# xxlong0/NeuralUDF

Measured on AMD Instinct MI355X. Metric: ray-samples/sec (train step), higher is better.
Workload: dtype f32 emulated on the 16-bit matrix pipe, f32 accumulate, f32 state / epilogues / optimizer.  Forward-order sweeps (UDF value, input gradient, colour / NeRF forward): f16x2 (x = hi + 2^-11 lo in fp16, 3 fp16 MFMA products, correction terms in their own accumulator).  Backward sweeps (tangent, adjoint

## Files before the change

### neuraludf_amd/csrc/gemm_tn_f32_mfma.hip

```cpp
#include "nudf_common.h"
#include "../../include/nudf.h"
#include <stdio.h>
#include <stdlib.h>
#include <string.h>
#include <type_traits>

#define BM 128
#define BN 128
#define BK 32
#define LDT (BM + 4)
#define T_TILE (BK * LDT)
#define TN_MAX_TILES 64
#define TN_WS_TILE (BM * BN + BM)
#define TNF_RETIRED (2 | 4)
#define TNF_NO_EPILOGUE 2
#define TNF_NO_BIAS 4
#define TNF_ATOMICS 8
#define TNF_UNIFORM_CHUNKS 16
#define TNF_NO_QUADRANTS 32
#define TNF_NO_XCD_MAP 64
#define TNF_NO_INTERLEAVE 128
#define TNF_NO_PACK16 256
#define TNF_NO_SPLIT_IMAGE 512
#define TNF_GENERIC_STAGE 2048
#define TNF_WIDE 1024

typedef float f32x8 __attribute__((ext_vector_type(8)));
typedef __bf16 bf16x8 __attribute__((ext_vector_type(8)));

struct TnTile {
  int blk_start;
  int rows_per_block;
  short prob, ti, tj;
  short layout;
  short n;
  short gfirst;
  short gn;
  short rot;
  int grid_start;
};
struct TnPlan {
  NudfGemmTNProblem prob[NUDF_TN_MAX_PROBLEMS];
  TnTile tile[TN_MAX_TILES + 1];
  int n_tiles, M, prec, flags;
  int grid_blocks;
  short partner[TN_MAX_TILES];
  int assign;
  int wide;
  short unit_tile[TN_MAX_TILES];
  int n_units, unit_chunks;
  float* ws;
  long long* dbg;
  const float* amax_a;
  const float* amax_b;
};

static_assert(sizeof(TnPlan) <= 4096, "TnPlan is passed by value: kernel arguments are limited to 4 KB");

__device__ __forceinline__ int tn_isub(int layout, int wave, int s) {
  return layout == 0 ? s : layout == 1 ? wave : (wave >> 1) * 2 + (s >> 1);
}
__device__ __forceinline__ int tn_jsub(int layout, int wave, int s) {
  return layout == 0 ? wave : layout == 1 ? s : (wave & 1) * 2 + (s & 1);
}

__host__ __device__ __forceinline__ void tn_decode_block(const TnPlan& g, int block, int& t, int& chunk) {
  int gf = 0;
  while (gf + g.tile[gf].gn < g.n_tiles && g.tile[gf + g.tile[gf].gn].grid_start <= block) gf += g.tile[gf].gn;
  const int T = g.tile[gf].gn;
  const int o = block - g.tile[gf].grid_start;
  t = gf;
  chunk = o;
  if (T > 1) {
    const int C = g.tile[gf + 1].blk_start - g.tile[gf].blk_start;
    const int c_hi = o / (8 * T), rem = o - c_hi * 8 * T;
    chunk = c_hi * 8 + (((rem & 7) - g.tile[gf].rot) & 7);
    t = chunk < C ? gf + (rem >> 3) : -1;
  }
}
__device__ __forceinline__ void tn_decode(const TnPlan& g, int& t, int& chunk) { tn_decode_block(g, (int)blockIdx.x, t, chunk); }

__global__ __launch_bounds__(256, 2) void gemm_tn_group_kernel(TnPlan g) {
  __shared__ __attribute__((aligned(16))) float smem[4 * T_TILE];
  float* As = smem;
  float* Bs = smem + 2 * T_TILE;

  const long long t_begin = g.dbg ? (long long)wall_clock64() : 0;
  const long long c_begin = g.dbg ? (long long)__builtin_amdgcn_s_memtime() : 0;
  int t, chunk;
  tn_decode(g, t, chunk);
  if (t < 0) return;
  const TnTile tl = g.tile[t];
  const NudfGemmTNProblem& q = g.prob[tl.prob];
  const int slot_id = tl.blk_start + chunk;

  const int tid = threadIdx.x;
  const int lane = tid & 63;
  const int wave = tid >> 6;
  const int i0 = tl.ti * BM, j0 = tl.tj * BN;
  const int lda = q.lda1, ldb = q.ldb1;
  const int mbeg = chunk * tl.rows_per_block;
  const int mend = min(mbeg + tl.rows_per_block, g.M);
  const int nk = (mend - mbeg + BK - 1) / BK;
  const int nfull = (mend - mbeg) / BK;

  const bool a16 = (q.flags & NUDF_TN_A16) != 0, b16 = (q.flags & NUDF_TN_B16) != 0;
  struct Op { const char* p; size_t rowb, stepb; unsigned poff[4]; int tk, tc, lds_pass; bool blk; };
  auto mk = [&](const float* base, int ld, int c0, bool h, bool blk) {
    Op o;
    const int esz = h ? 2 : 4;
    o.rowb = (size_t)ld * esz;
    o.stepb = (size_t)BK * o.rowb;
    o.blk = blk;
    if (blk) {
      o.tk = tid & 31;
      o.tc = (tid >> 5) * 4;
      o.lds_pass = 32;
      o.p = reinterpret_cast<const char*>(base) + (size_t)mbeg * o.rowb + (size_t)o.tk * 16;
#pragma unroll
      for (int ps = 0; ps < 4; ++ps) o.poff[ps] = (unsigned)(min(c0 + o.tc + 32 * ps, ld - 4) >> 2) * 512u;
    } else {
      o.tk = h ? tid >> 4 : tid >> 5;
      o.tc = h ? (tid & 15) * 8 : (tid & 31) * 4;
      o.lds_pass = (h ? 16 : 8) * LDT;
      const int col = min(c0 + o.tc, ld - (h ? 8 : 4));
      o.p = reinterpret_cast<const char*>(base) + (size_t)(mbeg + o.tk) * o.rowb + (size_t)col * esz;
#pragma unroll
      for (int ps = 0; ps < 4; ++ps) o.poff[ps] = (unsigned)((size_t)ps * (h ? 16 : 8) * o.rowb);
    }
    return o;
  };
  const Op oa = mk(q.A1, lda, i0, a16, (q.flags & NUDF_TN_A_BLK) != 0), ob = mk(q.B1, ldb, j0, b16, (q.flags & NUDF_TN_B_BLK) != 0);
  f32x4 ra[4], rb[4];
  int ld_rows = 0;
  auto load_op = [&](const Op& o, auto H, f32x4 (&r)[4], int kt, bool full) {
    constexpr bool h = decltype(H)::value;
    constexpr int np = h ? 2 : 4, rs = h ? 16 : 8;
    if (full || o.blk) {
      const char* b = o.p + (size_t)kt * o.stepb;
#pragma unroll
      for (int ps = 0; ps < np; ++ps) r[ps] = *reinterpret_cast<const f32x4*>(b + o.poff[ps]);
    } else {
#pragma unroll
      for (int ps = 0; ps < np; ++ps) {
        const ptrdiff_t row = min((ptrdiff_t)kt * BK + ps * rs, (ptrdiff_t)(g.M - 1 - mbeg - o.tk));
        r[ps] = *reinterpret_cast<const f32x4*>(o.p + row * (ptrdiff_t)o.rowb);
      }
    }
  };
  const bool do_bias = (q.dbias != nullptr) && (tl.tj == 0);
  f32x4 bacc = {0.f, 0.f, 0.f, 0.f}, bacc2 = {0.f, 0.f, 0.f, 0.f};
  f32x4 bacc3 = {0.f, 0.f, 0.f, 0.f}, bacc4 = {0.f, 0.f, 0.f, 0.f};
  auto widen = [](const f32x4& raw, f32x4& lo, f32x4& hi) {
    const uint4 u = __builtin_bit_cast(uint4, raw);
    lo = f32x4{__builtin_bit_cast(float, u.x << 16), __builtin_bit_cast(float, u.x & 0xffff0000u),
               __builtin_bit_cast(float, u.y << 16), __builtin_bit_cast(float, u.y & 0xffff0000u)};
    hi = f32x4{__builtin_bit_cast(float, u.z << 16), __builtin_bit_cast(float, u.z & 0xffff0000u),
               __builtin_bit_cast(float, u.w << 16), __builtin_bit_cast(float, u.w & 0xffff0000u)};
  };
  auto store_op = [&](const Op& o, auto H, const f32x4 (&r)[4], float* tile, bool bias) {
    constexpr bool h = decltype(H)::value;
    float* dst = tile + o.tk * LDT + o.tc;
    const f32x4 z = {0.f, 0.f, 0.f, 0.f};
    if constexpr (!h) {
      if (ld_rows >= BK) {
#pragma unroll
        for (int ps = 0; ps < 4; ++ps) *reinterpret_cast<f32x4*>(dst + ps * o.lds_pass) = r[ps];
        if (bias) {
          if (o.blk) { bacc += r[0]; bacc2 += r[1]; bacc3 += r[2]; bacc4 += r[3]; }
          else bacc += (r[0] + r[1]) + (r[2] + r[3]);
        }
        return;
      }
#pragma unroll
      for (int ps = 0; ps < 4; ++ps) {
        const f32x4 v = ((o.blk ? o.tk : ps * 8 + o.tk) < ld_rows) ? r[ps] : z;
        *reinterpret_cast<f32x4*>(dst + ps * o.lds_pass) = v;
        if (bias) {
// ... 1026 lines not shown
      const float x0 = (FULL || r0 + 2 * pp < mend) ? st[2 * pp] : 0.0f;
      const float x1 = (FULL || r0 + 2 * pp + 1 < mend) ? st[2 * pp + 1] : 0.0f;
      unsigned a, b;
      tn_split2_pair(x0, x1, scale, a, b);
      hq[pp >> 2][pp & 3] = a; lq[pp >> 2][pp & 3] = b;
      ps[pp] = x0 + x1;
    }
    if (bias) bias_acc += ((ps[0] + ps[1]) + (ps[2] + ps[3])) + ((ps[4] + ps[5]) + (ps[6] + ps[7]));
    unsigned* dst = tile + ((2 * sg) * 128 + sc) * 4;
    *reinterpret_cast<u32x4*>(dst) = hq[0];
    *reinterpret_cast<u32x4*>(dst + 512) = hq[1];
    *reinterpret_cast<u32x4*>(dst + T3Q) = lq[0];
    *reinterpret_cast<u32x4*>(dst + T3Q + 512) = lq[1];
  };
  auto mma = [&]() {
    const unsigned* as = As + ((lane >> 5) * 128 + (wave >> 1) * 64 + (lane & 31)) * 4;
    const unsigned* bs = Bs + ((lane >> 5) * 128 + (wave & 1) * 64 + (lane & 31)) * 4;
#pragma unroll
    for (int kk = 0; kk < BK3 / 16; ++kk) {
      u32x4 a[2][2], b[2][2];
#pragma unroll
      for (int s2 = 0; s2 < 2; ++s2)
#pragma unroll
        for (int pl = 0; pl < 2; ++pl) {
          a[s2][pl] = *reinterpret_cast<const u32x4*>(as + pl * T3Q + (2 * kk) * 512 + 128 * s2);
          b[s2][pl] = *reinterpret_cast<const u32x4*>(bs + pl * T3Q + (2 * kk) * 512 + 128 * s2);
        }
#pragma unroll
      for (int tt = 0; tt < 3; ++tt) {
        const int qa = (tt == 0) ? 1 : 0, qb = (tt == 1) ? 1 : 0;
#pragma unroll
        for (int j = 0; j < 2; ++j)
#pragma unroll
          for (int i = 0; i < 2; ++i) {
            if (tt < 2)
              acc1[i * 2 + j] = __builtin_amdgcn_mfma_f32_32x32x16_f16(__builtin_bit_cast(f16x8_t, a[i][qa]),
                                                                       __builtin_bit_cast(f16x8_t, b[j][qb]), acc1[i * 2 + j], 0, 0, 0);
            else
              acc[i * 2 + j] = __builtin_amdgcn_mfma_f32_32x32x16_f16(__builtin_bit_cast(f16x8_t, a[i][qa]),
                                                                      __builtin_bit_cast(f16x8_t, b[j][qb]), acc[i * 2 + j], 0, 0, 0);
          }
      }
    }
  };
  typedef std::integral_constant<bool, false> Ragged;
  typedef std::integral_constant<bool, true> Full;
  float sa[16], sb[16], sa2[16], sb2[16];
  if (nk > 0) {
    load(pa, lda, sa, 0);
    load(pb, ldb, sb, 0);
    if (nk > 1) {
      load(pa, lda, sa2, 1);
      load(pb, ldb, sb2, 1);
    }
    store(Ragged{}, sa, 0, As, sca, do_bias);
    store(Ragged{}, sb, 0, Bs, scb, false);
  }
  __syncthreads();
  auto kstep = [&](int kt, float (&la)[16], float (&lb)[16], float (&ua)[16], float (&ub)[16]) {
    if (kt + 2 < nk) {
      load(pa, lda, la, kt + 2);
      load(pb, ldb, lb, kt + 2);
    }
    __builtin_amdgcn_sched_barrier(0);
    mma();
    __builtin_amdgcn_sched_barrier(0);
    __syncthreads();
    if (kt + 1 < nk) {
      store(Ragged{}, ua, kt + 1, As, sca, do_bias);
      store(Ragged{}, ub, kt + 1, Bs, scb, false);
    }
    __syncthreads();
  };
  int kt0 = 0;
  {
    const bool last_ragged = ((mend - mbeg) % BK3) != 0 || mend > g.M;
    const int n_fast = nk - 2 - (last_ragged ? 1 : 0);
    if (n_fast >= 2 && (size_t)(g.M - mbeg) * (size_t)max(q.lda1, q.ldb1) * 4 < ((size_t)1 << 31)) {
      const int sgu = __builtin_amdgcn_readfirstlane(sg);
      const unsigned ca = (unsigned)min(i0 + sc, q.lda1 - 1), cbb = (unsigned)min(j0 + sc, q.ldb1 - 1);
      const __amdgpu_buffer_rsrc_t rsa = __builtin_amdgcn_make_buffer_rsrc(const_cast<float*>(q.A1 + (size_t)mbeg * lda), 0,
                                                                           (int)((size_t)(g.M - mbeg) * lda * 4), 0x00020000);
      const __amdgpu_buffer_rsrc_t rsb = __builtin_amdgcn_make_buffer_rsrc(const_cast<float*>(q.B1 + (size_t)mbeg * ldb), 0,
                                                                           (int)((size_t)(g.M - mbeg) * ldb * 4), 0x00020000);
      const int lda4 = q.lda1 * 4, ldb4 = q.ldb1 * 4;
      int ba = (2 * BK3 + 16 * sgu) * lda4, bb = (2 * BK3 + 16 * sgu) * ldb4;
      const int sa_step = BK3 * lda4, sb_step = BK3 * ldb4;
      auto load_f = [&](__amdgpu_buffer_rsrc_t rs, int so, int ld4, unsigned col, float (&st)[16]) {
#pragma unroll
        for (int r = 0; r < 16; ++r)
          st[r] = __builtin_bit_cast(float, __builtin_amdgcn_raw_buffer_load_b32(rs, (int)(col * 4), so + r * ld4, 0));
      };
      auto fstep = [&](float (&la)[16], float (&lb)[16], float (&ua)[16], float (&ub)[16]) {
        load_f(rsa, ba, lda4, ca, la);
        load_f(rsb, bb, ldb4, cbb, lb);
        ba += sa_step;
        bb += sb_step;
        __builtin_amdgcn_sched_barrier(0);
        mma();
        __builtin_amdgcn_sched_barrier(0);
        __syncthreads();
        store(Full{}, ua, 0, As, sca, do_bias);
        store(Full{}, ub, 0, Bs, scb, false);
        __syncthreads();
      };
      do {
        fstep(sa, sb, sa2, sb2);
        fstep(sa2, sb2, sa, sb);
        kt0 += 2;
      } while (kt0 + 1 < n_fast);
    }
  }
  for (int kt = kt0; kt < nk; kt += 2) {
    kstep(kt, sa, sb, sa2, sb2);
    if (kt + 1 < nk) kstep(kt + 1, sa2, sb2, sa, sb);
  }

  if (g.flags & TNF_NO_EPILOGUE) return;
  float* slot = g.ws ? g.ws + (size_t)slot_id * TN_WS_TILE : nullptr;
  if (do_bias) {
    float* red = reinterpret_cast<float*>(smem);
    red[sg * BM + sc] = bias_acc;
    __syncthreads();
    if (tid < BM) {
      const float sum = red[tid] + red[BM + tid];
      if (slot) slot[BM * BN + tid] = sum;
      else if (i0 + tid < q.NA) atomicAdd(q.dbias + i0 + tid, sum);
    }
  }
  const float unscale = inva * invb;
#pragma unroll
  for (int s4 = 0; s4 < 4; ++s4) {
#pragma unroll
    for (int r = 0; r < 16; ++r) acc[s4][r] = __builtin_fmaf(acc1[s4][r], 1.0f / 2048.0f, acc[s4][r]) * unscale;
    if (slot) {
      float* w = slot + ((wave * 4 + s4) * 64 + lane) * 16;
#pragma unroll
      for (int qd = 0; qd < 4; ++qd) {
        const f32x4 v = {acc[s4][4 * qd], acc[s4][4 * qd + 1], acc[s4][4 * qd + 2], acc[s4][4 * qd + 3]};
        *reinterpret_cast<f32x4*>(w + 4 * qd) = v;
      }
    } else {
      const int col = j0 + 32 * tn_jsub(2, wave, s4) + (lane & 31);
      if (col >= q.NB) continue;
#pragma unroll
      for (int r = 0; r < 16; ++r) {
        const int row = i0 + 32 * tn_isub(2, wave, s4) + (r & 3) + 8 * (r >> 2) + 4 * (lane >> 5);
        if (row < q.NA) atomicAdd(q.C + (size_t)row * q.ldc + col, acc[s4][r]);
      }
    }
  }
}

#define T3WA (4 * 256 * 4)
#define T3WB (4 * 128 * 4)
#define T3W_BUF (3 * T3WA + 3 * T3WB)
__global__ __launch_bounds__(512, 1) void gemm_tn3w_group_kernel(TnPlan g) {
  __shared__ __attribute__((aligned(16))) unsigned smem_w[2 * T3W_BUF];
  const int t = g.unit_tile[blockIdx.x / g.unit_chunks];
  const int chunk = blockIdx.x % g.unit_chunks;
  const int partner = g.partner[t];
  const TnTile tl = g.tile[t];
  const NudfGemmTNProblem& q = g.prob[tl.prob];
  const bool two = partner >= 0;
  const int slot0 = tl.blk_start + chunk;
  const int slot1 = two ? g.tile[partner].blk_start + chunk : slot0;

  const int tid = threadIdx.x;
  const int lane = tid & 63;
  const int wave = tid >> 6;
  const int i0 = tl.ti * BM, j0 = tl.tj * BN;
  const int mbeg = chunk * tl.rows_per_block;
  const int mend = min(mbeg + tl.rows_per_block, g.M);
  const int nk = (mend - mbeg + BK3 - 1) / BK3;
  const int sca = tid & 255, sga = tid >> 8;
  const int scb = tid & 127, sgb = tid >> 7;
  const bool bias_tile = (q.dbias != nullptr) && (tl.tj == 0) && !(g.flags & TNF_NO_BIAS);
  const bool do_bias = bias_tile && (two || sca < BM);
  float bias_acc = 0.0f;
  const bool mm_live = two || wave < 4;

  f32x16 acc[4];
#pragma unroll
  for (int s2 = 0; s2 < 4; ++s2)
#pragma unroll
    for (int r = 0; r < 16; ++r) acc[s2][r] = 0.0f;

  const float* pa = q.A1 + min(i0 + sca, q.lda1 - 1);
  const float* pb = q.B1 + min(j0 + scb, q.ldb1 - 1);
  const size_t lda = (size_t)q.lda1, ldb = (size_t)q.ldb1;
  auto load_a = [&](float (&st)[16], int kt) {
    const int r0 = mbeg + kt * BK3 + 16 * sga;
#pragma unroll
    for (int r = 0; r < 16; ++r) st[r] = pa[(size_t)min(r0 + r, g.M - 1) * lda];
  };
  auto load_b = [&](float (&st)[8], int kt) {
    const int r0 = mbeg + kt * BK3 + 8 * sgb;
#pragma unroll
    for (int r = 0; r < 8; ++r) st[r] = pb[(size_t)min(r0 + r, g.M - 1) * ldb];
  };
  auto store_a = [&](const float (&st)[16], int kt, unsigned* img) {
    const int r0 = mbeg + kt * BK3 + 16 * sga;
    u32x4 hq[2], mq[2], lq[2];
    float ps[8];
#pragma unroll
    for (int pp = 0; pp < 8; ++pp) {
      const float x0 = (r0 + 2 * pp < mend) ? st[2 * pp] : 0.0f;
      const float x1 = (r0 + 2 * pp + 1 < mend) ? st[2 * pp + 1] : 0.0f;
      unsigned a, b, d;
      tn_split3_pair(x0, x1, a, b, d);
      hq[pp >> 2][pp & 3] = a; mq[pp >> 2][pp & 3] = b; lq[pp >> 2][pp & 3] = d;
      ps[pp] = x0 + x1;
    }
    if (do_bias) bias_acc += ((ps[0] + ps[1]) + (ps[2] + ps[3])) + ((ps[4] + ps[5]) + (ps[6] + ps[7]));
    unsigned* dst = img + ((2 * sga) * 256 + sca) * 4;
    *reinterpret_cast<u32x4*>(dst) = hq[0];
    *reinterpret_cast<u32x4*>(dst + 1024) = hq[1];
    *reinterpret_cast<u32x4*>(dst + T3WA) = mq[0];
    *reinterpret_cast<u32x4*>(dst + T3WA + 1024) = mq[1];
    *reinterpret_cast<u32x4*>(dst + 2 * T3WA) = lq[0];
    *reinterpret_cast<u32x4*>(dst + 2 * T3WA + 1024) = lq[1];
  };
  auto store_b = [&](const float (&st)[8], int kt, unsigned* img) {
    const int r0 = mbeg + kt * BK3 + 8 * sgb;
    u32x4 hq, mq, lq;
#pragma unroll
    for (int pp = 0; pp < 4; ++pp) {
      const float x0 = (r0 + 2 * pp < mend) ? st[2 * pp] : 0.0f;
      const float x1 = (r0 + 2 * pp + 1 < mend) ? st[2 * pp + 1] : 0.0f;
      unsigned a, b, d;
      tn_split3_pair(x0, x1, a, b, d);
      hq[pp] = a; mq[pp] = b; lq[pp] = d;
    }
    unsigned* dst = img + 3 * T3WA + (sgb * 128 + scb) * 4;
    *reinterpret_cast<u32x4*>(dst) = hq;
    *reinterpret_cast<u32x4*>(dst + T3WB) = mq;
    *reinterpret_cast<u32x4*>(dst + 2 * T3WB) = lq;
  };
  auto mma = [&](const unsigned* img) {
    const unsigned* as = img + ((lane >> 5) * 256 + (wave >> 1) * 64 + (lane & 31)) * 4;
    const unsigned* bs = img + 3 * T3WA + ((lane >> 5) * 128 + (wave & 1) * 64 + (lane & 31)) * 4;
    u32x4 fa[2][2][3], fb[2][2][3];
    auto ldf = [&](int kk) {
#pragma unroll
      for (int s2 = 0; s2 < 2; ++s2)
#pragma unroll
        for (int pl = 0; pl < 3; ++pl) {
          fa[kk][s2][pl] = *reinterpret_cast<const u32x4*>(as + pl * T3WA + (2 * kk) * 1024 + 128 * s2);
          fb[kk][s2][pl] = *reinterpret_cast<const u32x4*>(bs + pl * T3WB + (2 * kk) * 512 + 128 * s2);
        }
    };
    ldf(0);
#pragma unroll
    for (int kk = 0; kk < BK3 / 16; ++kk) {
      if (kk + 1 < BK3 / 16) ldf(kk + 1);
      __builtin_amdgcn_sched_barrier(0);
#pragma unroll
      for (int tt = 0; tt < 6; ++tt) {
        const int qa = (tt == 0 || tt == 3 || tt == 5) ? 0 : (tt == 1 ? 2 : 1);
        const int qb = (tt == 0) ? 2 : ((tt == 2 || tt == 3) ? 1 : 0);
#pragma unroll
        for (int j = 0; j < 2; ++j)
#pragma unroll
          for (int i = 0; i < 2; ++i)
            acc[i * 2 + j] = __builtin_amdgcn_mfma_f32_32x32x16_bf16(__builtin_bit_cast(bf16x8, fa[kk][i][qa]),
                                                                     __builtin_bit_cast(bf16x8, fb[kk][j][qb]), acc[i * 2 + j], 0, 0, 0);
      }
      __builtin_amdgcn_sched_barrier(0);
    }
  };
  unsigned* buf0 = smem_w;
  unsigned* buf1 = smem_w + T3W_BUF;
  float sa[16], sb[8], sa2[16], sb2[8];
  if (nk > 0) {
    load_a(sa, 0);
    load_b(sb, 0);
    if (nk > 1) {
      load_a(sa2, 1);
      load_b(sb2, 1);
    }
    store_a(sa, 0, buf0);
    store_b(sb, 0, buf0);
  }
  const bool mma_first = wave < 4;
  long long tk_mma = 0, tk_store = 0, tk_load = 0, tk_bar = 0;
  const bool prof = g.dbg != nullptr;
  const long long tk_begin = prof ? (long long)__builtin_amdgcn_s_memtime() : 0;
#define TNW_STAMP(acc_) if (prof) { const long long n_ = (long long)__builtin_amdgcn_s_memtime(); acc_ += n_ - tk_last; tk_last = n_; }
  if (!mma_first && nk > 2) {
    load_a(sa, 2);
    load_b(sb, 2);
  }
  __syncthreads();
  auto kstep = [&](int kt, float (&la)[16], float (&lb)[8], float (&ua)[16], float (&ub)[8], const unsigned* cur, unsigned* nxt) {
    long long tk_last = prof ? (long long)__builtin_amdgcn_s_memtime() : 0;
    if (mma_first) {
      if (kt + 2 < nk) {
        load_a(la, kt + 2);
        load_b(lb, kt + 2);
      }
      __builtin_amdgcn_sched_barrier(0);
      TNW_STAMP(tk_load)
      if (mm_live) mma(cur);
      __builtin_amdgcn_sched_barrier(0);
      TNW_STAMP(tk_mma)
      if (kt + 1 < nk) {
        store_a(ua, kt + 1, nxt);
        store_b(ub, kt + 1, nxt);
      }
      __builtin_amdgcn_sched_barrier(0);
      TNW_STAMP(tk_store)
    } else {
      if (kt + 1 < nk) {
        store_a(ua, kt + 1, nxt);
        store_b(ub, kt + 1, nxt);
      }
      __builtin_amdgcn_sched_barrier(0);
      TNW_STAMP(tk_store)
      if (kt + 3 < nk) {
        load_a(ua, kt + 3);
        load_b(ub, kt + 3);
      }
      __builtin_amdgcn_sched_barrier(0);
      TNW_STAMP(tk_load)
      if (mm_live) mma(cur);
      __builtin_amdgcn_sched_barrier(0);
      TNW_STAMP(tk_mma)
    }
    __builtin_amdgcn_sched_barrier(0);
    __syncthreads();
    TNW_STAMP(tk_bar)
  };
  for (int kt = 0; kt < nk; kt += 2) {
    kstep(kt, sa, sb, sa2, sb2, buf0, buf1);
    if (kt + 1 < nk) kstep(kt + 1, sa2, sb2, sa, sb, buf1, buf0);
  }

#undef TNW_STAMP
  if (prof && lane == 0 && (wave == 0 || wave == 4)) {
    long long* d = g.dbg + 8 * (size_t)blockIdx.x + (wave ? 4 : 0);
    d[0] = ((long long)__builtin_amdgcn_s_memtime() - tk_begin) | ((long long)nk << 40);
    d[1] = tk_mma; d[2] = tk_store | (tk_load << 32); d[3] = tk_bar;
  }
  if (g.flags & TNF_NO_EPILOGUE) return;
  const int tsel = wave >> 2;
  const int vw = 2 * ((wave >> 1) & 1) + (wave & 1);
  float* slot_t[2] = {g.ws ? g.ws + (size_t)slot0 * TN_WS_TILE : nullptr, g.ws ? g.ws + (size_t)slot1 * TN_WS_TILE : nullptr};
  if (bias_tile) {
    float* red = reinterpret_cast<float*>(smem_w);
    red[sga * 256 + sca] = bias_acc;
    __syncthreads();
    if (tid < 256 && (two || tid < BM)) {
      const float sum = red[tid] + red[256 + tid];
      float* sl = slot_t[tid >> 7];
      if (sl) sl[BM * BN + (tid & 127)] = sum;
      else if (i0 + tid < q.NA) atomicAdd(q.dbias + i0 + tid, sum);
    }
  }
  if (!mm_live) return;
#pragma unroll
  for (int s2 = 0; s2 < 4; ++s2) {
    float* slot = slot_t[tsel];
    if (slot) {
      float* w = slot + ((vw * 4 + s2) * 64 + lane) * 16;
#pragma unroll
      for (int qd = 0; qd < 4; ++qd) {
        const f32x4 v = {acc[s2][4 * qd], acc[s2][4 * qd + 1], acc[s2][4 * qd + 2], acc[s2][4 * qd + 3]};
        *reinterpret_cast<f32x4*>(w + 4 * qd) = v;
      }
    } else {
      const int col = j0 + 32 * tn_jsub(2, vw, s2) + (lane & 31);
      if (col >= q.NB) continue;
#pragma unroll
      for (int r = 0; r < 16; ++r) {
        const int row = i0 + 128 * tsel + 32 * tn_isub(2, vw, s2) + (r & 3) + 8 * (r >> 2) + 4 * (lane >> 5);
        if (row < q.NA) atomicAdd(q.C + (size_t)row * q.ldc + col, acc[s2][r]);
      }
    }
  }
}

static int g_tn_flags = -1;
extern "C" int nudf_set_tn_flags(int f) {
  const int old = g_tn_flags < 0 ? 0 : g_tn_flags;
  g_tn_flags = f & ~TNF_RETIRED;
  return old;
}
static long long* g_tn_dbg = nullptr;
extern "C" int nudf_set_tn_debug(void* buf) {
  g_tn_dbg = (long long*)buf;
  return 0;
}
static int tn_flags() {
  if (g_tn_flags < 0) { const char* e = getenv("NUDF_TN_FLAGS"); g_tn_flags = (e ? atoi(e) : 0) & ~TNF_RETIRED; }
  return g_tn_flags;
}

static double tn_cost(int n) {
  static double c[4] = {-1.0, 0, 0, 0};
  if (c[0] < 0) {
    double d[4] = {2.0, 3.0, 3.5, 4.0};
    const char* e = getenv("NUDF_TN_COSTS");
    if (e) sscanf(e, "%lf,%lf,%lf,%lf", &d[0], &d[1], &d[2], &d[3]);
    for (int i = 3; i >= 0; --i) c[i] = d[i];
  }
  return c[n - 1];
}

static int tn_plan(const NudfGemmTNGroup& g, TnPlan& pl) {
  if (g.n_problems <= 0 || g.M <= 0) return 0;
  if (g.n_problems > NUDF_TN_MAX_PROBLEMS) {
    nudf_set_error("nudf_gemm_tn_grouped: too many problems", hipErrorInvalidValue);
    return -1;
  }
  const int flags = tn_flags();
  double cost[TN_MAX_TILES];
  int nt = 0;
  for (int i = 0; i < g.n_problems; ++i) {
    const NudfGemmTNProblem& q = g.prob[i];
    const int ma = (q.flags & NUDF_TN_A16) ? 8 : 4, mb = (q.flags & NUDF_TN_B16) ? 8 : 4;
    {
      const bool ap4 = (q.flags & NUDF_TN_A_P4) != 0, bp4 = (q.flags & NUDF_TN_B_P4) != 0;
      const bool a16 = (q.flags & NUDF_TN_A16) != 0, b16 = (q.flags & NUDF_TN_B16) != 0;
      if ((ap4 && !a16) || (bp4 && !b16) || ((ap4 || bp4) && (g.prec == 0 || g.prec == 3)) || (ap4 && b16 && !bp4) || (bp4 && a16 && !ap4) ||
          ((ap4 || bp4) && (flags & TNF_NO_PACK16)) || ((ap4 || bp4) && g.rows_per_block % 4)) {
        nudf_set_error("nudf_gemm_tn_grouped: a 4-point packed operand is a bf16 operand of the 16-bit MFMA mode "
                       "(NUDF_TN_x16 set, prec != 0, rows_per_block a multiple of 4); a problem's other operand is packed "
                       "as well or fp32", hipErrorInvalidValue);
        return -1;
      }
    }
    if (((q.flags & NUDF_TN_A_BLK) && (q.flags & NUDF_TN_A16)) || ((q.flags & NUDF_TN_B_BLK) && (q.flags & NUDF_TN_B16))) {
      nudf_set_error("nudf_gemm_tn_grouped: the blocked layout is defined for fp32 operands", hipErrorInvalidValue);
      return -1;
    }
    if ((q.lda1 % ma) || (q.ldb1 % mb) || q.NA <= 0 || q.NB <= 0 || q.lda1 < ma || q.ldb1 < mb ||
        (((uintptr_t)q.A1) & 15) || (((uintptr_t)q.B1) & 15)) {
      nudf_set_error("nudf_gemm_tn_grouped: leading dimensions must be multiples of 4, operands 16-byte aligned",
                     hipErrorInvalidValue);
      return -1;
    }
    pl.prob[i] = q;
    const int ti_n = (q.NA + BM - 1) / BM, tj_n = (q.NB + BN - 1) / BN;
    for (int ti = 0; ti < ti_n; ++ti)
      for (int tj = 0; tj < tj_n; ++tj) {
        if (nt >= TN_MAX_TILES) {
          nudf_set_error("nudf_gemm_tn_grouped: more than 64 output tiles of 128 x 128 in one group",
                         hipErrorInvalidValue);
          return -1;
        }
        int li = (q.NA - ti * BM + 31) / 32, lj = (q.NB - tj * BN + 31) / 32;
        if (li > 4) li = 4;
        if (lj > 4) lj = 4;
        TnTile& tl = pl.tile[nt];
        tl.prob = (short)i; tl.ti = (short)ti; tl.tj = (short)tj; tl.rot = 0;
        tl.layout = (short)(li <= lj ? 0 : 1);
        tl.n = (short)(li <= lj ? li : lj);
        if (li == 4 && lj == 4 && !(flags & TNF_NO_QUADRANTS)) tl.layout = 2;
        if (g.prec != 0 || (q.flags & (NUDF_TN_A16 | NUDF_TN_B16))) {
          tl.layout = 2;
          tl.n = 4;
        }
        cost[nt++] = tn_cost(tl.n);
      }
  }
  if (g.workspace && !(flags & TNF_ATOMICS)) {
    for (int i = 0; i < g.n_problems; ++i)
      for (int j = i + 1; j < g.n_problems; ++j) {
        const NudfGemmTNProblem &a = g.prob[i], &b = g.prob[j];
        const float *a0 = a.C, *a1 = a.C + (size_t)(a.NA - 1) * a.ldc + a.NB;
        const float *b0 = b.C, *b1 = b.C + (size_t)(b.NA - 1) * b.ldc + b.NB;
        const bool c_overlap = a0 < b1 && b0 < a1;
        const bool d_overlap = a.dbias && b.dbias && a.dbias < b.dbias + b.NA && b.dbias < a.dbias + a.NA;
        if (c_overlap || d_overlap) {
          nudf_set_error("nudf_gemm_tn_grouped: with a workspace the problems of a group must write disjoint C / dbias "
                         "ranges (the fixed-order reduction is not atomic)", hipErrorInvalidValue);
          return -1;
        }
      }
  }
  pl.n_tiles = nt;
  pl.M = g.M;
  pl.prec = g.prec;
  pl.flags = flags;
  pl.wide = 0;
  int n_units = nt;
  for (int t = 0; t < nt; ++t) pl.partner[t] = -1;
  {
    bool ok = g.prec == 3 && (flags & TNF_WIDE) && !(flags & TNF_NO_SPLIT_IMAGE);
    for (int i = 0; i < g.n_problems && ok; ++i)
      if (g.prob[i].flags & (NUDF_TN_A16 | NUDF_TN_B16 | NUDF_TN_A_BLK | NUDF_TN_B_BLK | NUDF_TN_A_P4 | NUDF_TN_B_P4)) ok = false;
    if (ok) {
      int pairs = 0;
      for (int t = 0; t < nt; ++t) {
        if (pl.partner[t] != -1 || (pl.tile[t].ti & 1)) continue;
        const NudfGemmTNProblem& q = g.prob[pl.tile[t].prob];
        const int tj_n = (q.NB + BN - 1) / BN;
        const int u = t + tj_n;
        if (u < nt && pl.tile[u].prob == pl.tile[t].prob && pl.tile[u].ti == pl.tile[t].ti + 1 && pl.tile[u].tj == pl.tile[t].tj) {
          pl.partner[t] = (short)u;
          pl.partner[u] = -2;
          ++pairs;
        }
      }
      if (4 * pairs >= nt) {
        pl.wide = 1;
        n_units = nt - pairs;
      } else {
        for (int t = 0; t < nt; ++t) pl.partner[t] = -1;
      }
    }
  }
  const int nkt = (g.M + BK - 1) / BK;
  int chunks_of[TN_MAX_TILES];
  int blocks = 0;
  auto layout = [&]() {
    blocks = 0;
    for (int t = 0; t < nt; ++t) {
      pl.tile[t].blk_start = blocks;
      blocks += (g.M + pl.tile[t].rows_per_block - 1) / pl.tile[t].rows_per_block;
    }
    pl.tile[nt].blk_start = blocks;
    pl.tile[nt].gfirst = (short)nt; pl.tile[nt].gn = 1; pl.tile[nt].rot = 0;
    for (int t = 0; t < nt;) {
      int e = t + 1;
      while (!(flags & TNF_NO_XCD_MAP) && e < nt && pl.tile[e].prob == pl.tile[t].prob &&
             pl.tile[e].rows_per_block == pl.tile[t].rows_per_block) ++e;
      for (int k = t; k < e; ++k) { pl.tile[k].gfirst = (short)t; pl.tile[k].gn = (short)(e - t); }
      t = e;
    }
    int load[8] = {0, 0, 0, 0, 0, 0, 0, 0};
    int G = 0;
    for (int t = 0; t < nt; t += pl.tile[t].gn) {
      const int T = pl.tile[t].gn, C = pl.tile[t + 1].blk_start - pl.tile[t].blk_start;
      int rot = 0, size = C;
      if (T == 1) {
        for (int i = 0; i < C; ++i) ++load[(G + i) & 7];
      } else {
        const int w = C & 7;
        for (int x = 0; x < 8; ++x) load[x] += T * (C >> 3);
        if (w) {
          int best = 1 << 30;
          for (int r = 0; r < 8; ++r) {
            int m = 0, sum = 0;
            for (int cl = 0; cl < w; ++cl) { const int l = load[(G + ((cl + r) & 7)) & 7]; m = l > m ? l : m; sum += l; }
            if (m * 4096 + sum < best) { best = m * 4096 + sum; rot = r; }
          }
          for (int cl = 0; cl < w; ++cl) load[(G + ((cl + rot) & 7)) & 7] += T;
        }
        size = ((C + 7) >> 3) * 8 * T;
      }
      for (int k = t; k < t + T; ++k) { pl.tile[k].grid_start = G; pl.tile[k].rot = (short)rot; }
      G += size;
    }
    pl.tile[nt].grid_start = G;
    pl.grid_blocks = G;
    int m = 0;
    for (int x = 0; x < 8; ++x) m = load[x] > m ? load[x] : m;
    return m;
  };
  if (g.rows_per_block > 0) {
    bool any_blk = false;
    for (int i = 0; i < g.n_problems; ++i) any_blk = any_blk || (g.prob[i].flags & (NUDF_TN_A_BLK | NUDF_TN_B_BLK));
    if (any_blk && (g.rows_per_block % 32)) {
      nudf_set_error("nudf_gemm_tn_grouped: rows_per_block must be a multiple of 32 with blocked operands",
                     hipErrorInvalidValue);
      return -1;
    }
    for (int t = 0; t < nt; ++t) pl.tile[t].rows_per_block = g.rows_per_block;
    layout();
  } else {
    static int target0 = -1;
    if (target0 < 0) { const char* e = getenv("NUDF_TNG_BLOCKS"); target0 = e ? atoi(e) : 512; }
    const int max_chunks = nkt / 8 > 0 ? nkt / 8 : 1;
    if (pl.wide) {
      static int target_w = -1;
      if (target_w < 0) { const char* e = getenv("NUDF_TNW_BLOCKS"); target_w = e ? atoi(e) : 256; }
      int n = target_w / n_units;
      if (n < 1) n = 1;
      if (n > max_chunks) n = max_chunks;
      for (int t = 0; t < nt; ++t) chunks_of[t] = n;
      for (int t = 0; t < nt; ++t) pl.tile[t].rows_per_block = ((nkt + chunks_of[t] - 1) / chunks_of[t]) * BK;
      layout();
    } else {
      for (int target = target0;; target -= 8) {
        auto count = [&](double T, bool store) {
          long total = 0;
          for (int t = 0; t < nt; ++t) {
            const double c = ((flags & TNF_UNIFORM_CHUNKS) || g.prec != 0) ? 4.0 : cost[t];
            long n = (long)((c * (double)nkt + T - 1e-9) / T);
            if (n < 1) n = 1;
            if (n > max_chunks) n = max_chunks;
            if (store) chunks_of[t] = (int)n;
            total += n;
          }
          return total;
        };
        double lo = 0.0, hi = 4.0 * nkt;
        if (count(hi, false) <= target) {
          for (int it = 0; it < 60; ++it) {
            const double mid = 0.5 * (lo + hi);
            if (count(mid, false) <= target) hi = mid; else lo = mid;
          }
        }
        count(hi, true);
        for (int t = 0; t < nt; ++t) pl.tile[t].rows_per_block = ((nkt + chunks_of[t] - 1) / chunks_of[t]) * BK;
        const int most = layout();
        if (most <= target0 / 8 || target - 8 < nt || target - 8 < target0 / 2) break;
      }
    }
  }
  pl.n_units = 0;
  pl.unit_chunks = nt > 0 ? pl.tile[1].blk_start - pl.tile[0].blk_start : 1;
  if (pl.wide) {
    for (int t = 0; t < nt; ++t) {
      if (pl.tile[t + 1].blk_start - pl.tile[t].blk_start != pl.unit_chunks) pl.wide = 0;
      if (pl.partner[t] != -2) pl.unit_tile[pl.n_units++] = (short)t;
    }
  }
  return blocks;
}

extern "C" int64_t nudf_gemm_tn_grouped_workspace(const NudfGemmTNGroup* args) {
  TnPlan pl;
  const int blocks = tn_plan(*args, pl);
  pl.dbg = nullptr;
  return blocks <= 0 ? (int64_t)blocks : (int64_t)blocks * TN_WS_TILE;
}

extern "C" int nudf_gemm_tn_grouped_plan(const NudfGemmTNGroup* args, int32_t* out, int capacity) {
  TnPlan pl;
  const int blocks = tn_plan(*args, pl);
  if (blocks <= 0) return blocks;
  for (int b = 0; b < pl.grid_blocks && b < capacity; ++b) {
    int t, chunk;
    tn_decode_block(pl, b, t, chunk);
    if (t < 0) { out[4 * b] = out[4 * b + 1] = out[4 * b + 2] = out[4 * b + 3] = -1; continue; }
    out[4 * b] = pl.tile[t].prob;
    out[4 * b + 1] = pl.tile[t].ti * 256 + pl.tile[t].tj;
    out[4 * b + 2] = chunk;
    out[4 * b + 3] = pl.tile[t].blk_start + chunk;
  }
  return pl.grid_blocks;
}

extern "C" int nudf_gemm_tn_grouped(const NudfGemmTNGroup* args, void* stream) {
  TnPlan pl;
  const int blocks = tn_plan(*args, pl);
  if (blocks == 0) return 0;
  if (blocks < 0) return (int)hipErrorInvalidValue;
  pl.ws = (pl.flags & TNF_ATOMICS) ? nullptr : args->workspace;
  pl.dbg = g_tn_dbg;
  pl.assign = args->assign ? 1 : 0;
  if (pl.assign && !pl.ws) {
    nudf_set_error("nudf_gemm_tn_grouped: assign needs the workspace (two-pass) path", hipErrorInvalidValue);
    return (int)hipErrorInvalidValue;
  }
  if (pl.ws && ((((uintptr_t)pl.ws) & 15) || args->workspace_floats < (int64_t)blocks * TN_WS_TILE)) {
    nudf_set_error("nudf_gemm_tn_grouped: workspace too small or not 16-byte aligned "
                   "(nudf_gemm_tn_grouped_workspace gives the size)", hipErrorInvalidValue);
    return (int)hipErrorInvalidValue;
  }
  bool packed16 = pl.prec != 0 && pl.prec != 3 && !(pl.flags & TNF_NO_PACK16);
  int n16 = 0;
  for (int i = 0; i < args->n_problems && packed16; ++i) {
    const int f = args->prob[i].flags;
    if (f & (NUDF_TN_A_BLK | NUDF_TN_B_BLK)) packed16 = false;
    n16 += ((f & NUDF_TN_A16) ? 1 : 0) + ((f & NUDF_TN_B16) ? 1 : 0);
  }
  if (n16 < args->n_problems) packed16 = false;
  bool any_p4 = false;
  for (int i = 0; i < args->n_problems; ++i) any_p4 = any_p4 || (args->prob[i].flags & (NUDF_TN_A_P4 | NUDF_TN_B_P4));
  if (any_p4) {
    for (int i = 0; i < args->n_problems; ++i)
      if (args->prob[i].flags & (NUDF_TN_A_BLK | NUDF_TN_B_BLK)) {
        nudf_set_error("nudf_gemm_tn_grouped: 4-point packed and blocked operands cannot share a group", hipErrorInvalidValue);
        return (int)hipErrorInvalidValue;
      }
    packed16 = true;
  }
  if (pl.prec == 4) {
    for (int i = 0; i < args->n_problems; ++i)
      if (args->prob[i].flags & (NUDF_TN_A16 | NUDF_TN_B16 | NUDF_TN_A_BLK | NUDF_TN_B_BLK | NUDF_TN_A_P4 | NUDF_TN_B_P4)) {
        nudf_set_error("nudf_gemm_tn_grouped: prec 4 (f16x2) takes fp32 row-major operands", hipErrorInvalidValue);
        return (int)hipErrorInvalidValue;
      }
    pl.amax_a = args->amax_a;
    pl.amax_b = args->amax_b;
    hipLaunchKernelGGL(gemm_tn2_group_kernel, dim3(pl.grid_blocks), dim3(256), 0, (hipStream_t)stream, pl);
    NUDF_CHECK_LAUNCH("nudf_gemm_tn_grouped");
    if (pl.ws) {
      hipLaunchKernelGGL(tn_reduce_kernel, dim3(pl.n_tiles * 17), dim3(256), 0, (hipStream_t)stream, pl);
      NUDF_CHECK_LAUNCH("nudf_gemm_tn_grouped (reduce)");
    }
    return 0;
  }
  bool split3 = pl.prec == 3 && !(pl.flags & TNF_NO_SPLIT_IMAGE);
  for (int i = 0; i < args->n_problems && split3; ++i)
    if (args->prob[i].flags & (NUDF_TN_A16 | NUDF_TN_B16 | NUDF_TN_A_BLK | NUDF_TN_B_BLK | NUDF_TN_A_P4 | NUDF_TN_B_P4)) split3 = false;
  if (split3 && pl.wide)
    hipLaunchKernelGGL(gemm_tn3w_group_kernel, dim3(pl.n_units * pl.unit_chunks), dim3(512), 0, (hipStream_t)stream, pl);
  else if (split3) hipLaunchKernelGGL(gemm_tn3_group_kernel, dim3(pl.grid_blocks), dim3(256), 0, (hipStream_t)stream, pl);
  else if (packed16) hipLaunchKernelGGL(gemm_tn16_group_kernel, dim3(pl.grid_blocks), dim3(256), 0, (hipStream_t)stream, pl);
  else hipLaunchKernelGGL(gemm_tn_group_kernel, dim3(pl.grid_blocks), dim3(256), 0, (hipStream_t)stream, pl);
  NUDF_CHECK_LAUNCH("nudf_gemm_tn_grouped");
  if (pl.ws) {
    hipLaunchKernelGGL(tn_reduce_kernel, dim3(pl.n_tiles * 17), dim3(256), 0, (hipStream_t)stream, pl);
    NUDF_CHECK_LAUNCH("nudf_gemm_tn_grouped (reduce)");
  }
  return 0;
}

extern "C" int nudf_gemm_tn(const NudfGemmTN* args, void* stream) {
  const NudfGemmTN& p = *args;
  if (p.M <= 0 || p.NA <= 0 || p.NB <= 0) return 0;
  NudfGemmTNGroup g;
  memset(&g, 0, sizeof(g));
  g.M = p.M; g.rows_per_block = p.rows_per_block; g.prec = p.prec;
  g.n_problems = p.A2 ? 2 : 1;
  NudfGemmTNProblem& q0 = g.prob[0];
  q0.A1 = p.A1; q0.B1 = p.B1; q0.C = p.C; q0.dbias = p.dbias;
  q0.lda1 = p.lda1; q0.ldb1 = p.ldb1; q0.ldc = p.ldc; q0.NA = p.NA; q0.NB = p.NB;
  if (p.A2) {
    NudfGemmTNProblem& q1 = g.prob[1];
    q1 = q0;
    q1.A1 = p.A2; q1.B1 = p.B2; q1.lda1 = p.lda2; q1.ldb1 = p.ldb2; q1.dbias = nullptr;
  }
  return nudf_gemm_tn_grouped(&g, stream);
}
```

Measured before the change: 19.29 million.

## Add wide f16x2 TN GEMM kernel with buffer loads and transposed LDS reads

Adds a new kernel for the f16x2 (prec 4) weight-gradient TN GEMM. Waves are specialised: half split the A operand into fp16 hi/lo planes and half split B, staging them in a swizzled LDS image. Fragments are read back with ds_read_tr16 transposed loads and fed to 32x32x16 f16 MFMAs, with register double-buffering of global buffer loads. The launcher uses this kernel by default when alignment and size limits allow, keeping the old kernel behind a NARROW flag. The validator now also accepts unaligned leading dimensions for prec 4, which the new kernel rejects and sends back to the old path. The added LDS, register pressure and swizzle logic may lower occupancy.

New measurement: 19.40 million (median of 6 runs). No clear change (+0.6%).

```diff
diff --git a/neuraludf_amd/csrc/gemm_tn_f32_mfma.hip b/neuraludf_amd/csrc/gemm_tn_f32_mfma.hip
--- a/neuraludf_amd/csrc/gemm_tn_f32_mfma.hip
+++ b/neuraludf_amd/csrc/gemm_tn_f32_mfma.hip
@@ -24,6 +24,7 @@
 #define TNF_NO_SPLIT_IMAGE 512
 #define TNF_GENERIC_STAGE 2048
 #define TNF_WIDE 1024
+#define TNF_TN2_NARROW 4096
 
 typedef float f32x8 __attribute__((ext_vector_type(8)));
 typedef __bf16 bf16x8 __attribute__((ext_vector_type(8)));
@@ -1356,6 +1357,197 @@
   }
 }
 
+typedef short s16x4 __attribute__((ext_vector_type(4)));
+typedef short s16x8 __attribute__((ext_vector_type(8)));
+typedef unsigned u32x2_t __attribute__((ext_vector_type(2)));
+typedef __attribute__((address_space(3))) s16x4 lds_s16x4;
+__global__ __launch_bounds__(256, 2) void gemm_tn2w_group_kernel(TnPlan g) {
+  constexpr int BKW = 32;
+  constexpr int PLANE = BKW * 256;
+  __shared__ __attribute__((aligned(16))) unsigned char smem[4 * PLANE];
+  unsigned char* As = smem;
+  unsigned char* Bs = smem + 2 * PLANE;
+
+  int t, chunk;
+  tn_decode(g, t, chunk);
+  if (t < 0) return;
+  const TnTile tl = g.tile[t];
+  const NudfGemmTNProblem& q = g.prob[tl.prob];
+  const int slot_id = tl.blk_start + chunk;
+
+  const int tid = threadIdx.x;
+  const int lane = tid & 63;
+  const int wave = tid >> 6;
+  const int i0 = tl.ti * BM, j0 = tl.tj * BN;
+  const int mbeg = chunk * tl.rows_per_block;
+  const int mend = min(mbeg + tl.rows_per_block, g.M);
+  const int nk = (mend - mbeg + BKW - 1) / BKW;
+  const int c4 = tid & 31, hh = lane >> 5;
+  const int wu = __builtin_amdgcn_readfirstlane(wave);
+  const bool opb = wu >= 2;
+  const int wh = wu & 1;
+  const bool tile_bias = (q.dbias != nullptr) && (tl.tj == 0);
+  const bool do_bias = tile_bias && !opb;
+  f32x4 bias_acc = {0.0f, 0.0f, 0.0f, 0.0f};
+  float sca, inva, scb, invb;
+  tn_scale_of(g.amax_a, sca, inva);
+  tn_scale_of(g.amax_b, scb, invb);
+  const float scale = opb ? scb : sca;
+
+  f32x16 acc[4], acc1[4];
+#pragma unroll
+  for (int s4 = 0; s4 < 4; ++s4)
+#pragma unroll
+    for (int r = 0; r < 16; ++r) { acc[s4][r] = 0.0f; acc1[s4][r] = 0.0f; }
+
+  const int ldo = opb ? q.ldb1 : q.lda1;
+  const int ld4 = ldo * 4;
+  const int col4 = min((opb ? j0 : i0) + 4 * c4, ldo - 4) * 4;
+  const __amdgpu_buffer_rsrc_t rs = __builtin_amdgcn_make_buffer_rsrc(const_cast<float*>((opb ? q.B1 : q.A1) + (size_t)mbeg * ldo), 0,
+                                                                      (int)((size_t)(g.M - mbeg) * ld4), 0x00020000);
+  const int rw0 = 16 * wh + 8 * hh;
+  auto load = [&](f32x4 (&st)[8], int kt) {
+#pragma unroll
+    for (int pp = 0; pp < 8; ++pp) {
+      const int r = min(kt * BKW + rw0 + pp, g.M - 1 - mbeg);
+      st[pp] = __builtin_bit_cast(f32x4, __builtin_amdgcn_raw_buffer_load_b128(rs, r * ld4 + col4, 0, 0));
+    }
+  };
+  const int vo = hh * 8 * ld4 + col4;
+  auto load_f = [&](int so, f32x4 (&st)[8]) {
+#pragma unroll
+    for (int pp = 0; pp < 8; ++pp)
+      st[pp] = __builtin_bit_cast(f32x4, __builtin_amdgcn_raw_buffer_load_b128(rs, vo, so + pp * ld4, 0));
+  };
+  unsigned char* img = smem + (opb ? 2 * PLANE : 0) + rw0 * 256 + (c4 & 7) * 8;
+  auto store = [&](auto FULLc, const f32x4 (&st)[8], int kt) {
+    constexpr bool FULL = decltype(FULLc)::value;
+    const int r0 = mbeg + kt * BKW + rw0;
+    f32x4 x[8];
+#pragma unroll
+    for (int pp = 0; pp < 8; ++pp) {
+      x[pp] = st[pp];
+      if (!FULL && r0 + pp >= mend) x[pp] = f32x4{0.0f, 0.0f, 0.0f, 0.0f};
+      unsigned h01, l01, h23, l23;
+      tn_split2_pair(x[pp][0], x[pp][1], scale, h01, l01);
+      tn_split2_pair(x[pp][2], x[pp][3], scale, h23, l23);
+      unsigned char* dst = img + pp * 256 + (((c4 >> 3) ^ (pp & 3)) * 64);
+      *reinterpret_cast<u32x2_t*>(dst) = u32x2_t{h01, h23};
+      *reinterpret_cast<u32x2_t*>(dst + PLANE) = u32x2_t{l01, l23};
+    }
+    if (do_bias) {
+      const f32x4 node = ((x[0] + x[1]) + (x[2] + x[3])) + ((x[4] + x[5]) + (x[6] + x[7]));
+      f32x4 other;
+#pragma unroll
+      for (int e = 0; e < 4; ++e) other[e] = __shfl_xor(node[e], 32);
+      bias_acc += node + other;
+    }
+  };
+  auto mma = [&]() {
+    const int qr = (lane >> 2) & 3;
+    const int rd = (8 * (lane >> 5) + qr) * 256 + ((lane >> 4) & 1) * 32 + (lane & 3) * 8;
+    const unsigned char* ab[2];
+    const unsigned char* bb[2];
+#pragma unroll
+    for (int s2 = 0; s2 < 2; ++s2) {
+      ab[s2] = As + rd + ((((wave >> 1) * 2 + s2) ^ qr) * 64);
+      bb[s2] = Bs + rd + ((((wave & 1) * 2 + s2) ^ qr) * 64);
+    }
+    auto frag = [&](const unsigned char* p) {
+      const s16x4 v0 = __builtin_amdgcn_ds_read_tr16_b64_v4i16((lds_s16x4*)(p));
+      const s16x4 v1 = __builtin_amdgcn_ds_read_tr16_b64_v4i16((lds_s16x4*)(p + 4 * 256));
+      return __builtin_bit_cast(f16x8_t, __builtin_shufflevector(v0, v1, 0, 1, 2, 3, 4, 5, 6, 7));
+    };
+#pragma unroll
+    for (int kk = 0; kk < BKW / 16; ++kk) {
+      f16x8_t a[2][2], b[2][2];
+#pragma unroll
+      for (int s2 = 0; s2 < 2; ++s2)
+#pragma unroll
+        for (int pl = 0; pl < 2; ++pl) {
+          a[s2][pl] = frag(ab[s2] + pl * PLANE + kk * 16 * 256);
+          b[s2][pl] = frag(bb[s2] + pl * PLANE + kk * 16 * 256);
+        }
+#pragma unroll
+      for (int tt = 0; tt < 3; ++tt) {
+        const int qa = (tt == 0) ? 1 : 0, qb = (tt == 1) ? 1 : 0;
+#pragma unroll
+        for (int j = 0; j < 2; ++j)
+#pragma unroll
+          for (int i = 0; i < 2; ++i) {
+            if (tt < 2) acc1[i * 2 + j] = __builtin_amdgcn_mfma_f32_32x32x16_f16(a[i][qa], b[j][qb], acc1[i * 2 + j], 0, 0, 0);
+            else acc[i * 2 + j] = __builtin_amdgcn_mfma_f32_32x32x16_f16(a[i][qa], b[j][qb], acc[i * 2 + j], 0, 0, 0);
+          }
+      }
+    }
+  };
+  typedef std::integral_constant<bool, false> Ragged;
+  typedef std::integral_constant<bool, true> Full;
+  f32x4 st[8];
+  if (nk > 0) {
+    load(st, 0);
+    store(Ragged{}, st, 0);
+    if (nk > 1) load(st, 1);
+  }
+  __syncthreads();
+  int kt = 0;
+  {
+    const int n_full = (mend - mbeg) / BKW;
+    int so = (2 * BKW + 16 * wh) * ld4;
+    for (; kt + 2 < n_full; ++kt) {
+      mma();
+      __builtin_amdgcn_sched_barrier(0);
+      __syncthreads();
+      store(Full{}, st, 0);
+      load_f(so, st);
+      so += BKW * ld4;
+      __syncthreads();
+    }
+  }
+  for (; kt < nk; ++kt) {
+    mma();
+    __builtin_amdgcn_sched_barrier(0);
+    __syncthreads();
+    if (kt + 1 < nk) store(Ragged{}, st, kt + 1);
+    if (kt + 2 < nk) load(st, kt + 2);
+    __syncthreads();
+  }
+
+  float* slot = g.ws ? g.ws + (size_t)slot_id * TN_WS_TILE : nullptr;
+  if (tile_bias) {
+    float* red = reinterpret_cast<float*>(smem);
+    if (!opb && hh == 0) *reinterpret_cast<f32x4*>(red + wh * BM + 4 * c4) = bias_acc;
+    __syncthreads();
+    if (tid < BM) {
+      const float sum = red[tid] + red[BM + tid];
+      if (slot) slot[BM * BN + tid] = sum;
+      else if (i0 + tid < q.NA) atomicAdd(q.dbias + i0 + tid, sum);
+    }
+  }
+  const float unscale = inva * invb;
+#pragma unroll
+  for (int s4 = 0; s4 < 4; ++s4) {
+#pragma unroll
+    for (int r = 0; r < 16; ++r) acc[s4][r] = __builtin_fmaf(acc1[s4][r], 1.0f / 2048.0f, acc[s4][r]) * unscale;
+    if (slot) {
+      float* w = slot + ((wave * 4 + s4) * 64 + lane) * 16;
+#pragma unroll
+      for (int qd = 0; qd < 4; ++qd) {
+        const f32x4 v = {acc[s4][4 * qd], acc[s4][4 * qd + 1], acc[s4][4 * qd + 2], acc[s4][4 * qd + 3]};
+        *reinterpret_cast<f32x4*>(w + 4 * qd) = v;
+      }
+    } else {
+      const int col = j0 + 32 * tn_jsub(2, wave, s4) + (lane & 31);
+      if (col >= q.NB) continue;
+#pragma unroll
+      for (int r = 0; r < 16; ++r) {
+        const int row = i0 + 32 * tn_isub(2, wave, s4) + (r & 3) + 8 * (r >> 2) + 4 * (lane >> 5);
+        if (row < q.NA) atomicAdd(q.C + (size_t)row * q.ldc + col, acc[s4][r]);
+      }
+    }
+  }
+}
+
 #define T3WA (4 * 256 * 4)
 #define T3WB (4 * 128 * 4)
 #define T3W_BUF (3 * T3WA + 3 * T3WB)
@@ -1638,8 +1830,10 @@
       nudf_set_error("nudf_gemm_tn_grouped: the blocked layout is defined for fp32 operands", hipErrorInvalidValue);
       return -1;
     }
-    if ((q.lda1 % ma) || (q.ldb1 % mb) || q.NA <= 0 || q.NB <= 0 || q.lda1 < ma || q.ldb1 < mb ||
-        (((uintptr_t)q.A1) & 15) || (((uintptr_t)q.B1) & 15)) {
+    const bool any_ld = g.prec == 4 && !(q.flags & (NUDF_TN_A16 | NUDF_TN_B16 | NUDF_TN_A_BLK | NUDF_TN_B_BLK));
+    if (any_ld ? (q.NA <= 0 || q.NB <= 0 || q.lda1 < 1 || q.ldb1 < 1 || ((((uintptr_t)q.A1) | ((uintptr_t)q.B1)) & 3))
+               : ((q.lda1 % ma) || (q.ldb1 % mb) || q.NA <= 0 || q.NB <= 0 || q.lda1 < ma || q.ldb1 < mb ||
+                  (((uintptr_t)q.A1) & 15) || (((uintptr_t)q.B1) & 15))) {
       nudf_set_error("nudf_gemm_tn_grouped: leading dimensions must be multiples of 4, operands 16-byte aligned",
                      hipErrorInvalidValue);
       return -1;
@@ -1891,7 +2085,15 @@
       }
     pl.amax_a = args->amax_a;
     pl.amax_b = args->amax_b;
-    hipLaunchKernelGGL(gemm_tn2_group_kernel, dim3(pl.grid_blocks), dim3(256), 0, (hipStream_t)stream, pl);
+    bool wide = !(pl.flags & TNF_TN2_NARROW);
+    for (int i = 0; i < args->n_problems && wide; ++i) {
+      const NudfGemmTNProblem& q = args->prob[i];
+      if ((((uintptr_t)q.A1 | (uintptr_t)q.B1) & 15) || q.lda1 < 4 || q.ldb1 < 4 || ((q.lda1 | q.ldb1) & 3) ||
+          (size_t)args->M * (size_t)(q.lda1 > q.ldb1 ? q.lda1 : q.ldb1) * 4 >= ((size_t)1 << 31))
+        wide = false;
+    }
+    if (wide) hipLaunchKernelGGL(gemm_tn2w_group_kernel, dim3(pl.grid_blocks), dim3(256), 0, (hipStream_t)stream, pl);
+    else hipLaunchKernelGGL(gemm_tn2_group_kernel, dim3(pl.grid_blocks), dim3(256), 0, (hipStream_t)stream, pl);
     NUDF_CHECK_LAUNCH("nudf_gemm_tn_grouped");
     if (pl.ws) {
       hipLaunchKernelGGL(tn_reduce_kernel, dim3(pl.n_tiles * 17), dim3(256), 0, (hipStream_t)stream, pl);
```
